# williamyang1991/VToonify

Measured on AMD Instinct MI355X. Metric: frames/sec at 1024x1024 VToonify-D inference, higher is better.
Workload: dtype bf16

## Files before the change

vtoonify_amd/csrc/style_ops.hip:

```cpp
#include "vt_common.hpp"

namespace {

__global__ void __launch_bounds__(256)
linear_kernel(float* __restrict__ y, int ld_y, const float* __restrict__ x, int ld_x,
              const float* __restrict__ W, const float* __restrict__ b, int rows, int in_dim,
              int out_dim, float w_scale, float b_scale, int act, float slope, float gain) {
    const int lane = threadIdx.x & 63;
    const int64_t wave = (int64_t)blockIdx.x * 4 + (threadIdx.x >> 6);
    const int64_t total = (int64_t)rows * out_dim;
    const int64_t wi = wave < total ? wave : total - 1;
    const int r = (int)(wi / out_dim), o = (int)(wi % out_dim);
    const float* xr = x + (int64_t)r * ld_x;
    const float* wr = W + (int64_t)o * in_dim;
    float acc = 0.0f;
    for (int i = lane; i < in_dim; i += 64) acc += xr[i] * wr[i];
    acc = wave_sum(acc);
    if (lane == 0 && wave < total) {
        float v = acc * w_scale;
        if (b) v += b[o] * b_scale;
        if (act == VT_ACT_LRELU) v = ((v > 0.0f) ? v : v * slope) * gain;
        else if (act == VT_ACT_SIGMOID) v = 1.0f / (1.0f + expf(-v));
        y[(int64_t)r * ld_y + o] = v;
    }
}

__global__ void __launch_bounds__(256)
pixel_norm_kernel(float* __restrict__ y, const float* __restrict__ x, int rows, int dim, const int* __restrict__ gate) {
    if (gate && gate[0] == 0) return;
    const int lane = threadIdx.x & 63;
    const int wave = blockIdx.x * 4 + (threadIdx.x >> 6);
    const int r = wave < rows ? wave : rows - 1;
    const float* xr = x + (int64_t)r * dim;
    float ss = 0.0f;
    for (int i = lane; i < dim; i += 64) ss += xr[i] * xr[i];
    ss = wave_sum(ss);
    const float inv = rsqrtf(ss / (float)dim + 1e-8f);
    if (wave < rows)
        for (int i = lane; i < dim; i += 64) y[(int64_t)r * dim + i] = xr[i] * inv;
}

template <typename T>
__global__ void __launch_bounds__(256)
modulate_weight_kernel(T* __restrict__ out, const float* __restrict__ w, const float* __restrict__ s,
                       int cout, int cin, int k, float scale, int demodulate,
                       const float* __restrict__ fir) {
    const int lane = threadIdx.x & 63;
    const int wave = blockIdx.x * 4 + (threadIdx.x >> 6);
    const int co = wave < cout ? wave : cout - 1;
    const bool live = wave < cout;
    const int taps = k * k;
    const int n = cin * taps;
    const float* wc = w + (int64_t)co * n;
    float demod = 1.0f;
    if (demodulate) {
        float ss = 0.0f;
        for (int i = lane; i < n; i += 64) {
            const float v = scale * wc[i] * s[i / taps];
            ss += v * v;
        }
        ss = wave_sum(ss);
        demod = rsqrtf(ss + 1e-8f);
    }
    if (!live) return;
    if (fir == nullptr) {
        T* oc = out + (int64_t)co * n;
        for (int i = lane; i < n; i += 64) {
            const int tap = i / cin, ci = i - tap * cin;
            const float v = scale * wc[ci * taps + tap] * s[ci] * demod;
            oc[i] = from_f32<T>(v);
        }
    } else {
        float K[16];
#pragma unroll
        for (int i = 0; i < 16; ++i) K[i] = fir[i];
        for (int ci = lane; ci < cin; ci += 64) {
            float wm[9];
#pragma unroll
            for (int t = 0; t < 9; ++t) wm[t] = scale * wc[ci * 9 + t] * s[ci] * demod;
#pragma unroll
            for (int p = 0; p < 4; ++p) {
                const int py = p >> 1, px = p & 1;
#pragma unroll
                for (int ky = 0; ky < 3; ++ky)
#pragma unroll
                    for (int kx = 0; kx < 3; ++kx) {
                        float acc = 0.0f;
#pragma unroll
                        for (int a = 0; a < 3; ++a) {
                            const int u = 4 - 2 * ky - a + py;
                            if (u < 0 || u > 3) continue;
#pragma unroll
                            for (int b = 0; b < 3; ++b) {
                                const int v = 4 - 2 * kx - b + px;
                                if (v < 0 || v > 3) continue;
                                acc += wm[a * 3 + b] * K[u * 4 + v];
                            }
                        }
                        out[((int64_t)(p * cout + co) * 9 + (ky * 3 + kx)) * cin + ci] = from_f32<T>(acc);
                    }
            }
        }
    }
}

constexpr int LIN_BATCH = 24, MOD_BATCH = 16;

struct LinearTable {
    vt_linear_item it[LIN_BATCH];
    const int* gate;
    int32_t first_wave[LIN_BATCH + 1];
    int32_t n;
};

__global__ void __launch_bounds__(256) linear_batch_kernel(const LinearTable t) {
    if (t.gate && t.gate[0] == 0) return;
    constexpr int RB = 6;
    const int lane = threadIdx.x & 63;
    const int wave = blockIdx.x * 4 + (threadIdx.x >> 6);
    __shared__ int pre[LIN_BATCH + 1];
    if (threadIdx.x <= (unsigned)t.n) pre[threadIdx.x] = t.first_wave[threadIdx.x];
    __syncthreads();
    const int total = pre[t.n];
    const int wv = wave < total ? wave : total - 1;
    int lo = 0, hi = t.n;
    while (hi - lo > 1) {
        const int mid = (lo + hi) >> 1;
        if (wv >= pre[mid]) lo = mid;
        else hi = mid;
    }
    const int k = lo;
    const vt_linear_item& L = t.it[k];
    const int o = wv - t.first_wave[k];
    const float* wr = L.W + (int64_t)o * L.in_dim;
    const bool quad = (L.in_dim % 4 == 0);
    const bool w16 = quad && ((uintptr_t)L.W % 16 == 0);
    const bool x16 = quad && (L.ld_x % 4 == 0) && ((uintptr_t)L.x % 16 == 0);
    for (int r0 = 0; r0 < L.rows; r0 += RB) {
        float acc[RB];
#pragma unroll
        for (int j = 0; j < RB; ++j) acc[j] = 0.0f;
        if (quad) {
            for (int i = lane * 4; i < L.in_dim; i += 256) {
                float w4[4];
                if (w16) {
                    unpack16<float>(ld128(wr + i), w4);
                } else {
                    w4[0] = wr[i]; w4[1] = wr[i + 1]; w4[2] = wr[i + 2]; w4[3] = wr[i + 3];
                }
#pragma unroll
                for (int j = 0; j < RB; ++j) {
                    const int r = (r0 + j < L.rows) ? r0 + j : L.rows - 1;
                    const float* xp = L.x + (int64_t)r * L.ld_x + i;
                    float x4[4];
                    if (x16) {
                        unpack16<float>(ld128(xp), x4);
                    } else {
                        x4[0] = xp[0]; x4[1] = xp[1]; x4[2] = xp[2]; x4[3] = xp[3];
                    }
                    acc[j] += (x4[0] * w4[0] + x4[1] * w4[1]) + (x4[2] * w4[2] + x4[3] * w4[3]);
                }
            }
        } else {
            for (int i = lane; i < L.in_dim; i += 64) {
                const float w = wr[i];
#pragma unroll
                for (int j = 0; j < RB; ++j) {
                    const int r = (r0 + j < L.rows) ? r0 + j : L.rows - 1;
                    acc[j] += L.x[(int64_t)r * L.ld_x + i] * w;
                }
            }
        }
#pragma unroll
        for (int j = 0; j < RB; ++j) acc[j] = wave_sum(acc[j]);
        if (lane == 0 && wave < total) {
#pragma unroll
            for (int j = 0; j < RB; ++j) {
                if (r0 + j >= L.rows) break;
                float v = acc[j] * L.w_scale;
                if (L.b) v += L.b[o] * L.b_scale;
                if (L.act == VT_ACT_LRELU) v = ((v > 0.0f) ? v : v * L.slope) * L.gain;
                else if (L.act == VT_ACT_SIGMOID) v = 1.0f / (1.0f + expf(-v));
                L.y[(int64_t)(r0 + j) * L.ld_y + o] = v;
            }
        }
    }
}

struct ModTable {
    vt_modulate_item it[MOD_BATCH];
    const int* gate;
    int32_t first_row[MOD_BATCH + 1];
    int32_t n;
};

template <typename T>
__global__ void __launch_bounds__(256) modulate_batch_kernel(const ModTable t) {
    if (t.gate && t.gate[0] == 0) return;
    __shared__ float red[4];
    const int tid = threadIdx.x, lane = tid & 63, wv = tid >> 6;
    int lo = 0, hi = t.n;
    while (hi - lo > 1) {
        const int mid = (lo + hi) >> 1;
        if ((int)blockIdx.x >= t.first_row[mid]) lo = mid;
        else hi = mid;
    }
    const int k = lo;
    const vt_modulate_item& M = t.it[k];
    const int co = blockIdx.x - t.first_row[k];
    const int cout = M.cout, cin = M.cin, taps = M.k * M.k;
    const int n = cin * taps;
    const float* w = (const float*)M.weight;
    const float* s = M.s;
    const float* wc = w + (int64_t)co * n;
    const float scale = M.scale;
    float demod = 1.0f;
    if (M.demodulate) {
        float ss = 0.0f;
        for (int i = tid; i < n; i += 256) {
            const float v = scale * wc[i] * s[i / taps];
            ss += v * v;
        }
        ss = wave_sum(ss);
        if (lane == 0) red[wv] = ss;
        __syncthreads();
        demod = rsqrtf(((red[0] + red[1]) + (red[2] + red[3])) + 1e-8f);
    }
    T* out = (T*)M.out;
    if (M.fir == nullptr) {
        T* oc = out + (int64_t)co * n;
        for (int i = tid; i < n; i += 256) {
            const int tap = i / cin, ci = i - tap * cin;
            oc[i] = from_f32<T>(scale * wc[ci * taps + tap] * s[ci] * demod);
        }
    } else {
        float K[16];
#pragma unroll
        for (int i = 0; i < 16; ++i) K[i] = M.fir[i];
        for (int ci = tid; ci < cin; ci += 256) {
            float wm[9];
#pragma unroll
            for (int q = 0; q < 9; ++q) wm[q] = scale * wc[ci * 9 + q] * s[ci] * demod;
#pragma unroll
            for (int p = 0; p < 4; ++p) {
                const int py = p >> 1, px = p & 1;
#pragma unroll
                for (int ky = 0; ky < 3; ++ky)
#pragma unroll
                    for (int kx = 0; kx < 3; ++kx) {
                        float acc = 0.0f;
#pragma unroll
                        for (int a = 0; a < 3; ++a) {
                            const int u = 4 - 2 * ky - a + py;
                            if (u < 0 || u > 3) continue;
#pragma unroll
                            for (int b = 0; b < 3; ++b) {
                                const int v = 4 - 2 * kx - b + px;
                                if (v < 0 || v > 3) continue;
                                acc += wm[a * 3 + b] * K[u * 4 + v];
                            }
                        }
                        out[((int64_t)(p * cout + co) * 9 + (ky * 3 + kx)) * cin + ci] = from_f32<T>(acc);
                    }
            }
        }
    }
}

template <typename T>
__global__ void __launch_bounds__(256)
pack_weight_kernel(T* __restrict__ out, const float* __restrict__ w, int cout, int cin_src, int kh,
                   int kw, int cin_dst, const int32_t* __restrict__ chan_map, float scale,
                   int src_transposed) {
    const int taps = kh * kw;
    const int64_t total = (int64_t)cout * taps * cin_dst;
    const int64_t stride = (int64_t)gridDim.x * 256;
    for (int64_t i = (int64_t)blockIdx.x * 256 + threadIdx.x; i < total; i += stride) {
        const int cd = (int)(i % cin_dst);
        const int64_t t = i / cin_dst;
        const int tap = (int)(t % taps);
        const int co = (int)(t / taps);
        const int cs = chan_map ? chan_map[cd] : (cd < cin_src ? cd : -1);
        float v = 0.0f;
        if (cs >= 0) {
            if (!src_transposed) {
                v = w[((int64_t)co * cin_src + cs) * taps + tap];
            } else {
                v = w[((int64_t)cs * cout + co) * taps + tap];
            }
        }
        out[i] = from_f32<T>(v * scale);
    }
}

}

extern "C" int vt_linear(float* y, int ld_y, const float* x, int ld_x, const float* W,
                         const float* b, int rows, int in_dim, int out_dim, float w_scale,
                         float b_scale, int act, float slope, float gain, vt_stream stream) {
    VT_REQUIRE(y && x && W, "vt_linear: null tensor");
    VT_REQUIRE(rows >= 0 && in_dim > 0 && out_dim > 0, "vt_linear: bad sizes");
    VT_REQUIRE(act == VT_ACT_NONE || act == VT_ACT_LRELU || act == VT_ACT_SIGMOID, "vt_linear: unsupported act %d", act);
    if (rows == 0) return VT_OK;
    const int64_t waves = (int64_t)rows * out_dim;
    VT_LAUNCH(linear_kernel, dim3((unsigned)((waves + 3) / 4)), dim3(256), stream, y, ld_y, x, ld_x,
              W, b, rows, in_dim, out_dim, w_scale, b_scale, act, slope, gain);
    return vt_check_launch("vt_linear");
}

extern "C" int vt_pixel_norm(float* y, const float* x, int rows, int dim, vt_stream stream) {
    VT_REQUIRE(y && x && rows >= 0 && dim > 0, "vt_pixel_norm: bad arguments");
    if (rows == 0) return VT_OK;
    VT_LAUNCH(pixel_norm_kernel, dim3((unsigned)((rows + 3) / 4)), dim3(256), stream, y, x, rows, dim, (const int*)nullptr);
    return vt_check_launch("vt_pixel_norm");
}

extern "C" int vt_modulate_weight(void* out, const float* weight, const float* s, int cout, int cin,
                                  int k, float scale, int demodulate, const float* fir,
                                  int out_dtype, vt_stream stream) {
    VT_REQUIRE(out && weight && s, "vt_modulate_weight: null tensor");
    VT_REQUIRE(cout > 0 && cin > 0 && (k == 1 || k == 3), "vt_modulate_weight: bad shape");
    VT_REQUIRE(!fir || k == 3, "vt_modulate_weight: polyphase fold needs a 3x3 kernel");
    dim3 grid((unsigned)((cout + 3) / 4)), block(256);
    if (out_dtype == VT_F32) {
        auto kf = modulate_weight_kernel<float>;
        VT_LAUNCH(kf, grid, block, stream, (float*)out, weight, s, cout, cin, k, scale, demodulate, fir);
    } else if (out_dtype == VT_BF16) {
        auto kf = modulate_weight_kernel<bf16_t>;
        VT_LAUNCH(kf, grid, block, stream, (bf16_t*)out, weight, s, cout, cin, k, scale, demodulate, fir);
    } else if (out_dtype == VT_F16) {
        auto kf = modulate_weight_kernel<f16_t>;
        VT_LAUNCH(kf, grid, block, stream, (f16_t*)out, weight, s, cout, cin, k, scale, demodulate, fir);
    } else {
        vt_set_error("vt_modulate_weight: unsupported dtype %d", out_dtype);
        return VT_ERR_UNSUPPORTED;
    }
    return vt_check_launch("vt_modulate_weight");
}

extern "C" int vt_pack_conv_weight(void* out, const float* w, int cout, int cin_src, int kh, int kw,
                                   int cin_dst, const int32_t* chan_map, float scale,
                                   int src_transposed, int out_dtype, vt_stream stream) {
    VT_REQUIRE(out && w, "vt_pack_conv_weight: null tensor");
    VT_REQUIRE(cout > 0 && cin_src > 0 && cin_dst > 0 && kh > 0 && kw > 0, "vt_pack_conv_weight: bad shape");
    const int64_t total = (int64_t)cout * kh * kw * cin_dst;
    int64_t blocks = (total + 255) / 256;
    if (blocks > 8192) blocks = 8192;
    dim3 grid((unsigned)blocks), block(256);
    if (out_dtype == VT_F32) {
        auto kf = pack_weight_kernel<float>;
        VT_LAUNCH(kf, grid, block, stream, (float*)out, w, cout, cin_src, kh, kw, cin_dst, chan_map, scale, src_transposed);
    } else if (out_dtype == VT_BF16) {
        auto kf = pack_weight_kernel<bf16_t>;
        VT_LAUNCH(kf, grid, block, stream, (bf16_t*)out, w, cout, cin_src, kh, kw, cin_dst, chan_map, scale, src_transposed);
    } else if (out_dtype == VT_F16) {
        auto kf = pack_weight_kernel<f16_t>;
        VT_LAUNCH(kf, grid, block, stream, (f16_t*)out, w, cout, cin_src, kh, kw, cin_dst, chan_map, scale, src_transposed);
    } else {
        vt_set_error("vt_pack_conv_weight: unsupported dtype %d", out_dtype);
        return VT_ERR_UNSUPPORTED;
    }
    return vt_check_launch("vt_pack_conv_weight");
}

static int linear_batch_impl(const vt_linear_item* items, int n_items, const int* gate, vt_stream stream);
extern "C" int vt_linear_batch(const vt_linear_item* items, int n_items, vt_stream stream) {
    return linear_batch_impl(items, n_items, nullptr, stream);
}
// ... 110 lines not shown
```

vtoonify_amd/engine.py:

```python
from __future__ import annotations

import ctypes as C
import math
import os
from typing import Dict, List, Optional, Tuple

import torch

from . import _lib
from . import kernels as K
from ._lib import ACT_LRELU, ACT_NONE, ACT_RELU_TANH, OUT_NCHW, OUT_NHWC

SQRT2 = math.sqrt(2.0)
N_LATENT = 18
_DIL = {1: 4, 2: 4, 3: 2, 4: 2, 5: 1, 6: 1}
SKIP_HDR = 64


def _pad8(c: int) -> int:
    return (c + 7) // 8 * 8


class _Plan:
    def __init__(self):
        self.bufs: Dict[str, torch.Tensor] = {}
        self.style_ops: List[Tuple] = []
        self.enc_ops: List[Tuple] = []
        self.gen_ops: List[Tuple] = []
        self.keep: list = []
        self.masks: List[torch.Tensor] = []
        self.graphs: dict = {}
        self.convs: list = []


class VToonifyEngine:
    supports_borrow = True

    def __init__(self, state_dict: Dict[str, torch.Tensor], backbone: str = "dualstylegan",
                 in_size: int = 256, dtype: torch.dtype = torch.bfloat16,
                 device: Optional[torch.device] = None, cache_styles: bool = False,
                 tile_hints: Optional[Dict[str, int]] = None, style_gate: bool = False, x3: bool = False,
                 fuse_rgb128: bool = True, fused_gate=True, fold_rgb_up: bool = True):
        assert backbone in ("dualstylegan", "toonify")
        assert dtype in (torch.bfloat16, torch.float16, torch.float32)
        self.backbone = backbone
        self.dual = backbone == "dualstylegan"
        self.in_size = in_size
        self.dtype = dtype
        self.dt = K.dt_code(dtype)
        self.x3 = bool(x3) and dtype == torch.float32
        self.dt_conv = K.VT_F32X3 if self.x3 else self.dt
        self.h16 = dtype in (torch.bfloat16, torch.float16)
        self.precision = ({torch.bfloat16: "bf16", torch.float16: "fp16"}[dtype] if self.h16 else
                          ("fp32x3" if self.x3 else "fp32_exact"))
        self.esz = 2 if self.h16 else 4
        any_t = next(iter(state_dict.values()))
        self.device = torch.device(device) if device is not None else any_t.device
        if self.device.type == "cuda" and self.device.index is None:
            self.device = torch.device("cuda", torch.cuda.current_device())
        self.lib = _lib.lib()
        if self.device.type != "cuda" and not _lib.is_emulation():
            raise _lib.VtError("VToonifyEngine needs a GPU device (no CPU path)")
        self.cache_styles = cache_styles
        self.fuse_rgb128 = bool(fuse_rgb128)
        self.fused_gate = fused_gate if fused_gate == "all" else bool(fused_gate)
        self.fold_rgb_up = bool(fold_rgb_up)
        self.style_gate = bool(style_gate)
        self.graph_first = os.environ.get("VT_GRAPH_FIRST", "1") != "0"
        self.use_upblur = True
        self.tile_hints: Dict[str, int] = dict(tile_hints or {})
        if not self.tile_hints and os.environ.get("VT_TILE_HINTS"):
            import json
            with open(os.environ["VT_TILE_HINTS"]) as f:
                self.tile_hints = {k: int(v) for k, v in json.load(f).items()}
        self.sd = {k: v.detach().to(self.device, torch.float32).contiguous() for k, v in state_dict.items()}
        self.g = "generator.generator." if self.dual else "generator."
        self.n_down = 0
        while f"encoder.{self.n_down}.0.weight" in self.sd:
            self.n_down += 1
        self.n_fuse = sum(1 for lvl in range(5) if 2 ** (5 + lvl) <= in_size)
        import collections
        self._plans: "collections.OrderedDict[tuple, _Plan]" = collections.OrderedDict()
        self.max_plans = max(1, int(os.environ.get("VT_MAX_PLANS", "12")))
        self._shape_seen: Dict[tuple, int] = {}
        self._pack_static()

    def _pack_static(self):
        sd, T = self.sd, self.dtype
        self.w: Dict[str, torch.Tensor] = {}
        for bi in range(self.n_down):
            for j in (0, 2):
                wsrc = sd[f"encoder.{bi}.{j}.weight"]
                cin_dst = self._kpad(wsrc.shape[1]) if j == 2 else None
                if self._stem32(bi):
                    cin_dst = 32
                self.w[f"encoder.{bi}.{j}"] = K.pack_conv_weight(wsrc, cin_dst=cin_dst, out_dtype=T)
        for ii in range(6):
            for nm in ("conv", "conv2"):
                key = f"encoder.{self.n_down}.{ii}.{nm}"
                self.w[key] = K.pack_conv_weight(sd[key + ".weight"], out_dtype=T)
        self.w["enc_rgb"] = K.pack_conv_weight(sd[f"encoder.{self.n_down + 1}.weight"], out_dtype=T)
        if self.dual:
            for ii in range(1, 7):
                for nm in ("conv", "conv2"):
                    w = sd[f"res.{ii}.{nm}.0.weight"]
                    scale = 1.0 / math.sqrt(w.shape[1] * w.shape[2] * w.shape[3])
                    self.w[f"res.{ii}.{nm}"] = K.pack_conv_weight(w, scale=scale, out_dtype=T)
        for fi in range(self.n_fuse):
            if self.dual:
                self.w[f"fusion_out.{fi}.conv"] = K.pack_conv_weight(sd[f"fusion_out.{fi}.conv.weight"], out_dtype=T)
                self.w[f"fusion_out.{fi}.conv2"] = K.pack_conv_weight(sd[f"fusion_out.{fi}.conv2.weight"], out_dtype=T)
            else:
                self.w[f"fusion_out.{fi}"] = K.pack_conv_weight(sd[f"fusion_out.{fi}.weight"], out_dtype=T)
            wsk = sd[f"fusion_skip.{fi}.weight"]
            c = wsk.shape[1] - 3
            cmap = torch.tensor([0, 1, 2] + [-1] * (SKIP_HDR - 3) + list(range(3, c + 3)), dtype=torch.int32,
                                device=self.device)
            self.w[f"fusion_skip.{fi}"] = K.pack_conv_weight(wsk, cin_dst=c + SKIP_HDR, chan_map=cmap, out_dtype=T)
        self.modw = {}
        for i in range(6, 16):
            self.modw[f"convs.{i}"] = sd[f"{self.g}convs.{i}.conv.weight"][0].contiguous()
        for i in range(3, 8):
            self.modw[f"to_rgbs.{i}"] = sd[f"{self.g}to_rgbs.{i}.conv.weight"][0].contiguous()
            self.w[f"to_rgbs.{i}.bias"] = sd[f"{self.g}to_rgbs.{i}.bias"].reshape(3).contiguous()
        self.fir_up = sd[f"{self.g}convs.6.conv.blur.kernel"].contiguous()
        self.fir_rgb = sd[f"{self.g}to_rgbs.3.upsample.kernel"].contiguous()
        if self.use_upblur:
            k = self.fir_up.detach().float().cpu()
            if not (k.shape == (4, 4) and float(k.sum()) != 0.0 and
                    torch.allclose(torch.outer(k.sum(1), k.sum(0)) / k.sum(), k, rtol=1e-5, atol=1e-7)):
                self.use_upblur = False
        self._wstream: Dict[int, torch.Tensor] = {}
        unit = 8 * (64 if self.h16 else 32)
        for key, wt in self.w.items():
            if wt.ndim == 3 and wt.shape[1] == 9 and wt.shape[2] % unit == 0 and wt.shape[0] % 8 == 0:
                st = K.conv_weight_stream(wt)
                if st is not None:
                    self._wstream[wt.data_ptr()] = st

    def _stem32(self, bi: int) -> bool:
        sd = self.sd
        w0, w2 = sd[f"encoder.{bi}.0.weight"], sd[f"encoder.{bi}.2.weight"]
        return (bi == 0 and self.h16 and w0.shape[1] <= 32 and w0.shape[0] == 32 and
                w2.shape[0] % 32 == 0 and w2.shape[0] <= 256)

    def _kpad(self, c: int) -> int:
        step = 64 if self.h16 else 32
        return (c + step - 1) // step * step

    def _buf(self, plan: _Plan, name: str, shape, dtype=None) -> torch.Tensor:
        t = torch.empty(shape, dtype=dtype or self.dtype, device=self.device)
        plan.bufs[name] = t
        return t

    @staticmethod
    def conv_signature(d) -> str:
        return (f"{d.h}x{d.w}:{d.c0 + d.c1}->{d.cout * d.phases}:k{d.kh}s{d.stride}d{d.dil}p{d.phases}"
                + (":nchw" if d.out_layout == OUT_NCHW else "") + (":up" if d.up_fir else ""))

    def _apply_hint(self, d):
        h = self.tile_hints.get(self.conv_signature(d))
        if h:
            d.tile_hint = int(h)
        return d

    def _op_conv(self, ops, plan, ref_macs=None, branch=0, join=False, entry=None, **kw):
        wt = kw.get("weight")
        if isinstance(wt, torch.Tensor) and wt.data_ptr() in self._wstream:
            kw["weight_stream"] = self._wstream[wt.data_ptr()]
        d = self._apply_hint(K.make_conv_desc(dtype=self.dt_conv, **kw))
        plan.keep.append(d)
        cin = d.c0 + d.c1
        m = d.n * d.out_h * d.out_w
        cout_t = d.cout * d.phases
        macs = m * cout_t * d.kh * d.kw * cin if ref_macs is None else ref_macs
        osz = 4 if d.out_dtype == K.VT_F32 else 2
        nbytes = (d.n * d.h * d.w * cin * self.esz + cout_t * d.kh * d.kw * cin * self.esz +
                  m * cout_t * osz * (2 if d.resid else 1))
        info = {"name": "conv", "kernel": "conv_igemm", "flops": 2 * macs, "bytes": nbytes, "cin": cin,
                "cout": cout_t, "m": m, "k": d.kh * d.kw * cin, "hw": (d.out_h, d.out_w),
                "sig": self.conv_signature(d)}
        if branch:
            info["branch"] = branch
        if join:
            info["join"] = True
        if entry is not None:
            info["form"] = entry[2]
            info["bytes"] += entry[3]
        plan.convs.append((d, info, ops, len(ops)))
        ops.append((self.lib.vt_conv2d, (C.byref(d),), info) if entry is None else (entry[0], (C.byref(d),) + tuple(entry[1]), info))

    def _conv_kind(self, **kw) -> int:
        wt = kw.get("weight")
        if isinstance(wt, torch.Tensor) and wt.data_ptr() in self._wstream:
            kw["weight_stream"] = self._wstream[wt.data_ptr()]
        d = self._apply_hint(K.make_conv_desc(dtype=self.dt_conv, **kw))
        d.splitk_ws, d.splitk_ws_bytes = 1 << 20, 1 << 40
        tile = self.lib.vt_conv2d_tile(C.byref(d))
        return tile // 100000000 if tile >= 0 else -1

    def _rgbup_resident(self, tile: int, n: int, ho: int, wo: int, cout: int) -> bool:
        if os.environ.get("VT_PATCH_PIPE", "")[:1] in ("0", "1") or os.environ.get("VT_BATCH_EXACT", "")[:1] == "1":
            return False
        kind, sk, bm, bn = tile // 100000000, (tile // 1000000) % 100, (tile // 1000) % 1000, tile % 1000
        return (kind == 1 and sk <= 1 and bm == 256 and bn == 64 and cout == 64 and
                n * ((ho + 15) // 16) * ((wo + 15) // 16) >= 2 * self._patchw_wgs())

    def _patchw_wgs(self) -> int:
        e = os.environ.get("VT_PATCHW_WGS", "")
        if e.isdigit() and int(e) > 0:
            return int(e)
        if self.device.type == "cuda":
            return torch.cuda.get_device_properties(self.device).multi_processor_count
        return 256

    def _op_linear(self, ops, y, ld_y, x, ld_x, W, b, rows, w_scale=1.0, b_scale=1.0, act=ACT_NONE,
                   slope=0.2, gain=1.0):
        out_dim, in_dim = W.shape
        ops.append((self.lib.vt_linear,
                    (C.c_void_p(K._ptr(y)), ld_y, C.c_void_p(K._ptr(x)), ld_x, C.c_void_p(W.data_ptr()),
                     C.c_void_p(b.data_ptr() if b is not None else 0), rows, in_dim, out_dim,
                     float(w_scale), float(b_scale), act, float(slope), float(gain)), "linear"))

    @staticmethod
    def _info(what):
        if isinstance(what, dict):
            return what
        return {"name": what, "kernel": what, "flops": 0, "bytes": 0}

    def _run(self, ops, stream, plan=None):
        for fn, args, what in ops:
            rc = fn(*args, stream)
            if rc != 0:
                raise _lib.VtError(f"{self._info(what)['name']} failed (code {rc}): "
                                   f"{self.lib.vt_last_error().decode()}")

    def _build_style_ops(self, plan: _Plan, ns: int, has_res: bool):
        sd, g, ops, lib = self.sd, self.g, plan.style_ops, self.lib
        f32 = torch.float32
        style_in = self._buf(plan, "style_in", (ns, N_LATENT, 512), f32)
        gate = None
        if self.style_gate:
            style_in.zero_()
            style_new = self._buf(plan, "style_new", (ns, N_LATENT, 512), f32)
            gflag = self._buf(plan, "style_gate", (2,), torch.int32)
            gflag[0], gflag[1] = 0, 1
            gate = C.c_void_p(gflag.data_ptr())
            ops.append((lib.vt_style_gate, (gate, C.c_void_p(style_in.data_ptr()), C.c_void_p(style_new.data_ptr()),
                                            ns * N_LATENT * 512), "style_gate"))
        ada = self._buf(plan, "adastyles", (ns, N_LATENT, 512), f32)
        ds = self._buf(plan, "d_s", (1,), f32)
        rows = ns * N_LATENT
        levels: List[list] = [[] for _ in range(5)]

        def lin(level, y, ld_y, x, ld_x, W, b, nrows, w_scale=1.0, b_scale=1.0, act=ACT_NONE, slope=0.2,
                gain=1.0):
            it = _lib.LinearItem()
            it.y, it.x, it.W = K._ptr(y), K._ptr(x), W.data_ptr()
            it.b = b.data_ptr() if b is not None else None
            it.ld_y, it.ld_x, it.rows = ld_y, ld_x, nrows
            it.out_dim, it.in_dim = W.shape
            it.act, it.w_scale, it.b_scale, it.slope, it.gain = act, w_scale, b_scale, slope, gain
            levels[level].append(it)

        if self.dual:
            pn = self._buf(plan, "pn", (rows, 512), f32)
            t1 = self._buf(plan, "tc1", (rows, 512), f32)
            res = self._buf(plan, "resstyles", (ns, N_LATENT, 512), f32)
            if gate is not None:
                ops.append((lib.vt_pixel_norm_gated, (C.c_void_p(pn.data_ptr()), C.c_void_p(style_in.data_ptr()), rows, 512,
                                                      gate), "pixel_norm"))
            else:
                ops.append((lib.vt_pixel_norm, (C.c_void_p(pn.data_ptr()), C.c_void_p(style_in.data_ptr()), rows, 512),
                            "pixel_norm"))
            sc = (1.0 / math.sqrt(512)) * 0.01
            lin(0, t1, 512, pn, 512, sd["generator.style.1.weight"], sd["generator.style.1.bias"],
                rows, sc, 0.01, ACT_LRELU, 0.2, SQRT2)
            lin(1, res, 512, t1, 512, sd["generator.style.2.weight"], sd["generator.style.2.bias"],
                rows, sc, 0.01, ACT_LRELU, 0.2, SQRT2)
            for i in range(7, N_LATENT):
                lin(0, ada.data_ptr() + i * 512 * 4, N_LATENT * 512, style_in.data_ptr() + i * 512 * 4,
                    N_LATENT * 512, sd[f"generator.res.{i}.weight"], sd[f"generator.res.{i}.bias"], ns,
                    1.0 / math.sqrt(512), 1.0)
        else:
            ops.append((self._copy_op, (ada, style_in), "copy"))

        plan.modw = {}
        mods = []
        for lvl in range(5):
            for name, lat, demod, up in ((f"convs.{6 + 2 * lvl}", 7 + 2 * lvl, True, True),
                                         (f"convs.{7 + 2 * lvl}", 8 + 2 * lvl, True, False),
                                         (f"to_rgbs.{3 + lvl}", 9 + 2 * lvl, False, False)):
                w = self.modw[name]
                cout, cin, k, _ = w.shape
                s = self._buf(plan, f"s.{name}", (ns, cin), f32)
                lin(1, s, cin, ada.data_ptr() + lat * 512 * 4, N_LATENT * 512,
                    sd[f"{g}{name}.conv.modulation.weight"], sd[f"{g}{name}.conv.modulation.bias"],
                    ns, 1.0 / math.sqrt(512), 1.0)
                phases = 4 if (up and not self.use_upblur) else 1
                taps = 9 if up else k * k
                wm = self._buf(plan, f"wm.{name}", (ns, phases * cout, taps, cin))
                plan.modw[name] = wm
                for b in range(ns):
                    it = _lib.ModulateItem()
                    it.out = wm.data_ptr() + b * phases * cout * taps * cin * self.esz
                    it.weight, it.s = w.data_ptr(), s.data_ptr() + b * cin * 4
                    it.fir = self.fir_up.data_ptr() if (up and not self.use_upblur) else None
                    it.cout, it.cin, it.k, it.demodulate = cout, cin, k, int(demod)
                    it.scale = 1.0 / math.sqrt(cin * k * k)
                    mods.append(it)
        if self.dual:
            if has_res:
                for ii in range(1, 7):
                    for nm in ("norm", "norm2"):
                        Wl = sd[f"res.{ii}.{nm}.style.weight"]
                        gb = self._buf(plan, f"gb.res.{ii}.{nm}", (ns, Wl.shape[0]), f32)
                        lin(2, gb, Wl.shape[0], plan.bufs["resstyles"].data_ptr() + ii * 512 * 4,
                            N_LATENT * 512, Wl, sd[f"res.{ii}.{nm}.style.bias"], ns)
            for fi in range(self.n_fuse):
                p = f"fusion_out.{fi}."
                l0 = self._buf(plan, f"lab0.{fi}", (ns, 64), f32)
                l1 = self._buf(plan, f"lab1.{fi}", (ns, 128), f32)
                lin(0, l0, 64, ds, 0, sd[p + "linear.0.weight"], sd[p + "linear.0.bias"], ns,
                    1.0, 1.0, ACT_LRELU, 0.2, 1.0)
                lin(1, l1, 128, l0, 64, sd[p + "linear.2.weight"], sd[p + "linear.2.bias"], ns,
                    1.0, 1.0, ACT_LRELU, 0.2, 1.0)
                Wl = sd[p + "norm.style.weight"]
                gb = self._buf(plan, f"gb.fus.{fi}", (ns, Wl.shape[0]), f32)
                lin(2, gb, Wl.shape[0], l1, 128, Wl, sd[p + "norm.style.bias"], ns)
        else:
            pass
        for lv in levels:
            if not lv:
                continue
            arr = (_lib.LinearItem * len(lv))(*lv)
            plan.keep.append(arr)
            linfo = {"name": "linear", "kernel": "linear_batch", "flops": 0, "bytes": 0}
            if gate is not None:
                ops.append((lib.vt_linear_batch_gated, (arr, len(lv), gate), linfo))
            else:
                ops.append((lib.vt_linear_batch, (arr, len(lv)), linfo))
        marr = (_lib.ModulateItem * len(mods))(*mods)
        plan.keep.append(marr)
        minfo = {"name": "modulate", "kernel": "modulate_batch", "flops": 0,
                 "bytes": sum(m.cout * m.cin * m.k * m.k * (4 + self.esz * (4 if m.fir else 1)) for m in mods)}
        if gate is not None:
            ops.append((lib.vt_modulate_weight_batch_gated, (marr, len(mods), self.dt, gate), minfo))
        else:
            ops.append((lib.vt_modulate_weight_batch, (marr, len(mods), self.dt), minfo))

    @staticmethod
    def _copy_op(dst, src, stream):
        dst.copy_(src)
        return 0

    @staticmethod
    def _fill_rows_op(dst, src, stream):
        dst.copy_(src.expand_as(dst))
        return 0

    def _build_plan(self, B: int, H: int, W: int, shared: bool, has_res: bool) -> _Plan:
        sd, g, lib, dt = self.sd, self.g, self.lib, self.dt
        plan = _Plan()
        ns = 1 if shared else B
        self._build_style_ops(plan, ns, has_res)
        f32 = torch.float32
        ops = plan.enc_ops
        ds = plan.bufs["d_s"]

        cin0 = sd["encoder.0.0.weight"].shape[1]
        cin_p = 32 if self._stem32(0) else _pad8(cin0)
        x_nhwc = self._buf(plan, "x_nhwc", (B, H, W, cin_p))
        if cin_p != _pad8(cin0):
            x_nhwc.zero_()
        plan.cin0 = cin0
        cur, cc, h, w = x_nhwc, cin_p, H, W
        feats = []
        for bi in range(self.n_down):
            stride = 1 if bi == 0 else 2
            for j in (0, 2):
                wt = sd[f"encoder.{bi}.{j}.weight"]
                co = wt.shape[0]
                st = stride if j == 0 else 1
                ho, wo = (h + 2 - 3) // st + 1, (w + 2 - 3) // st + 1
                cs = self._kpad(co) if (j == 0 and not self._stem32(bi)) else co
                out = self._buf(plan, f"enc{bi}.{j}", (B, ho, wo, cs))
                if cs != co:
                    out.zero_()
                self._op_conv(ops, plan, src0=cur, c0=cc, ld0=cc, n=B, h=h, w=w, out_h=ho, out_w=wo,
                              weight=self.w[f"encoder.{bi}.{j}"], cout=co, kh=3, kw=3, stride=st, pad=1,
                              bias=sd[f"encoder.{bi}.{j}.bias"], act=ACT_LRELU, slope=0.2, out=out, ld_out=cs)
                cur, cc, h, w = out, cs, ho, wo
            feats.append((cur, cc, h, w))
        feats = feats[::-1]
        cf = cc
        tmp = self._buf(plan, "res_tmp", (B, h, w, cf))
        ping = [self._buf(plan, "feat_a", (B, h, w, cf)), self._buf(plan, "feat_b", (B, h, w, cf))]
        hw = h * w
        if self.dual and has_res:
            sc1 = self._buf(plan, "in_scale", (B, cf), f32)
            sh1 = self._buf(plan, "in_shift", (B, cf), f32)
            ws = self._buf(plan, "in_ws", (max(K.instnorm_ws_bytes(B, hw, cf), 16),), torch.uint8)
            nrm_res = self._buf(plan, "nrm_res", (B, h, w, cf))
        feat = cur
        pp = 0
        rk = f"encoder.{self.n_down}"
        plane_adain = self.dual and has_res and hw <= 4096
        for ii in range(6):
            self._op_conv(ops, plan, src0=feat, c0=cf, ld0=cf, n=B, h=h, w=w, out_h=h, out_w=w,
                          weight=self.w[f"{rk}.{ii}.conv"], cout=cf, kh=3, kw=3, pad=1,
                          bias=sd[f"{rk}.{ii}.conv.bias"], act=ACT_LRELU, out=tmp, ld_out=cf)
            nxt = ping[pp]; pp ^= 1
            self._op_conv(ops, plan, src0=tmp, c0=cf, ld0=cf, n=B, h=h, w=w, out_h=h, out_w=w,
                          weight=self.w[f"{rk}.{ii}.conv2"], cout=cf, kh=3, kw=3, pad=1,
                          bias=sd[f"{rk}.{ii}.conv2.bias"], act=ACT_LRELU, alpha=1 / SQRT2, beta=1 / SQRT2,
                          resid=feat, ld_res=cf, out=nxt, ld_out=cf,
                          stats_part=ws if (self.dual and has_res and hw <= 16384 and not plane_adain) else None)
            feat = nxt
            if plane_adain:
                r = ii + 1
                dil = _DIL[r]
                gb1, gb2 = plan.bufs[f"gb.res.{r}.norm"], plan.bufs[f"gb.res.{r}.norm2"]
                ldg = 0 if ns == 1 else gb1.shape[1]

                def _plane(dst, src, gb):
                    ops.append((lib.vt_instnorm_plane,
                                (C.c_void_p(dst.data_ptr()), cf, C.c_void_p(src.data_ptr()), cf, C.c_void_p(0), 0, B, hw, cf,
                                 C.c_void_p(gb.data_ptr()), ldg, dt),
                                {"name": "adain", "kernel": "instnorm_plane", "flops": 0,
                                 "bytes": 2 * B * hw * cf * self.esz}))
                _plane(nrm_res, feat, gb1)
                self._op_conv(ops, plan, src0=nrm_res, c0=cf, ld0=cf, n=B, h=h, w=w, out_h=h, out_w=w,
                              weight=self.w[f"res.{r}.conv"], cout=cf, kh=3, kw=3, pad=dil, dil=dil,
                              bias=sd[f"res.{r}.conv.1.bias"], act=ACT_LRELU, gain=SQRT2, out=tmp, ld_out=cf)
                _plane(tmp, tmp, gb2)
                nxt = ping[pp]; pp ^= 1
                self._op_conv(ops, plan, src0=tmp, c0=cf, ld0=cf, n=B, h=h, w=w, out_h=h, out_w=w,
                              weight=self.w[f"res.{r}.conv2"], cout=cf, kh=3, kw=3, pad=dil, dil=dil,
                              bias=sd[f"res.{r}.conv2.1.bias"], act=ACT_LRELU, gain=SQRT2, alpha_dev=ds, beta=1.0,
                              resid=feat, ld_res=cf, out=nxt, ld_out=cf)
                feat = nxt
            elif self.dual and has_res:
                r = ii + 1
                dil = _DIL[r]
                for nm, src, dst in (("norm", feat, tmp), ("norm2", tmp, None)):
                    gb = plan.bufs[f"gb.res.{r}.{nm}"]
                    if hw <= 16384:
                        ops.append((lib.vt_instnorm_apply_stats,
                                    (C.c_void_p(nrm_res.data_ptr()), cf, C.c_void_p(src.data_ptr()), cf, B, hw, cf,
                                     C.c_void_p(gb.data_ptr()), 0 if ns == 1 else gb.shape[1],
                                     C.c_void_p(ws.data_ptr()), dt),
                                    {"name": "adain", "kernel": "instnorm_apply", "flops": 0,
                                     "bytes": 2 * B * hw * cf * self.esz}))
                    else:
                        ops.append((lib.vt_instnorm_stats,
                                    (C.c_void_p(sc1.data_ptr()), C.c_void_p(sh1.data_ptr()), C.c_void_p(src.data_ptr()),
                                     cf, C.c_void_p(0), 0, B, hw, cf, C.c_void_p(gb.data_ptr()),
                                     0 if ns == 1 else gb.shape[1], C.c_void_p(ws.data_ptr()), dt),
                                    {"name": "instnorm", "kernel": "instnorm_stats", "flops": 0,
                                     "bytes": B * hw * cf * self.esz}))
                        ops.append((lib.vt_affine_apply,
                                    (C.c_void_p(nrm_res.data_ptr()), cf, C.c_void_p(src.data_ptr()), cf,
                                     C.c_void_p(0), 0, C.c_void_p(sc1.data_ptr()), C.c_void_p(sh1.data_ptr()),
                                     B, hw, cf, dt),
                                    {"name": "affine", "kernel": "affine_apply", "flops": 0,
                                     "bytes": 2 * B * hw * cf * self.esz}))
                    cn = "conv" if nm == "norm" else "conv2"
                    if dst is not None:
                        self._op_conv(ops, plan, src0=nrm_res, c0=cf, ld0=cf, n=B, h=h, w=w, out_h=h, out_w=w,
                                      weight=self.w[f"res.{r}.{cn}"], cout=cf, kh=3, kw=3, pad=dil, dil=dil,
                                      bias=sd[f"res.{r}.{cn}.1.bias"],
                                      act=ACT_LRELU, gain=SQRT2, out=dst, ld_out=cf,
                                      stats_part=ws if hw <= 16384 else None)
                    else:
                        nxt = ping[pp]; pp ^= 1
                        self._op_conv(ops, plan, src0=nrm_res, c0=cf, ld0=cf, n=B, h=h, w=w, out_h=h, out_w=w,
                                      weight=self.w[f"res.{r}.{cn}"], cout=cf, kh=3, kw=3, pad=dil, dil=dil,
                                      bias=sd[f"res.{r}.{cn}.1.bias"],
                                      act=ACT_LRELU, gain=SQRT2, alpha_dev=ds, beta=1.0, resid=feat, ld_res=cf,
                                      out=nxt, ld_out=cf)
                        feat = nxt
        plan.feat = (feat, cf, h, w)
        skip = self._buf(plan, "skip_enc", (B, 3, h, w), f32)
        self._op_conv(ops, plan, src0=feat, c0=cf, ld0=cf, n=B, h=h, w=w, out_h=h, out_w=w,
# ... 370 lines not shown
```

Baseline: 1691.

## Trim style MLP to used rows and restructure linear/modulate style kernels

The style mapping MLP (pixel norm plus two linears) now runs only over the latent rows that the residual blocks read, instead of all 18 rows per sample. It is also skipped entirely when no residual path needs it. The batched linear kernel keeps small weight rows in registers, adds a single-row specialization, and spreads the final per-row writes across lanes. The modulate kernel stages the scaled weights in shared memory so that non-FIR rows are read once for both the demod sum and the output. The style stage is cheap relative to the generator, so the overall effect on frame rate is likely small.

```diff
diff --git a/vtoonify_amd/csrc/style_ops.hip b/vtoonify_amd/csrc/style_ops.hip
--- a/vtoonify_amd/csrc/style_ops.hip
+++ b/vtoonify_amd/csrc/style_ops.hip
@@ -113,6 +113,93 @@
     int32_t n;
 };
 
+__device__ __forceinline__ float fmul(float a, float b) {
+#ifdef VT_EMU
+    return a * b;
+#else
+    return __fmul_rn(a, b);
+#endif
+}
+__device__ __forceinline__ float fadd(float a, float b) {
+#ifdef VT_EMU
+    return a + b;
+#else
+    return __fadd_rn(a, b);
+#endif
+}
+__device__ __forceinline__ float dot4(const float (&x)[4], const float (&w)[4]) {
+    return fadd(fadd(fmul(x[0], w[0]), fmul(x[1], w[1])), fadd(fmul(x[2], w[2]), fmul(x[3], w[3])));
+}
+__device__ __forceinline__ void ld_quad(float (&v)[4], const float* p, bool vec) {
+    if (vec) {
+        unpack16<float>(ld128(p), v);
+    } else {
+        v[0] = p[0]; v[1] = p[1]; v[2] = p[2]; v[3] = p[3];
+    }
+}
+
+template <int NR>
+__device__ __forceinline__ void linear_rows(const vt_linear_item& L, const float* wr, const float (&wq)[2][4], bool wregs,
+                                            float bias, int o, int r0, int lane, bool live, bool quad, bool w16, bool x16) {
+    float acc[NR];
+    const float* xr[NR];
+#pragma unroll
+    for (int j = 0; j < NR; ++j) {
+        acc[j] = 0.0f;
+        const int r = (r0 + j < L.rows) ? r0 + j : L.rows - 1;
+        xr[j] = L.x + (int64_t)r * L.ld_x;
+    }
+    if (wregs) {
+        float xq[2][NR][4];
+#pragma unroll
+        for (int s = 0; s < 2; ++s) {
+            const int i = lane * 4 + 256 * s;
+            if (i < L.in_dim) {
+#pragma unroll
+                for (int j = 0; j < NR; ++j) ld_quad(xq[s][j], xr[j] + i, x16);
+            }
+        }
+#pragma unroll
+        for (int s = 0; s < 2; ++s) {
+            if (lane * 4 + 256 * s < L.in_dim) {
+#pragma unroll
+                for (int j = 0; j < NR; ++j) acc[j] = fadd(acc[j], dot4(xq[s][j], wq[s]));
+            }
+        }
+    } else if (quad) {
+        for (int i = lane * 4; i < L.in_dim; i += 256) {
+            float w4[4], x4[NR][4];
+            ld_quad(w4, wr + i, w16);
+#pragma unroll
+            for (int j = 0; j < NR; ++j) ld_quad(x4[j], xr[j] + i, x16);
+#pragma unroll
+            for (int j = 0; j < NR; ++j) acc[j] = fadd(acc[j], dot4(x4[j], w4));
+        }
+    } else {
+        for (int i = lane; i < L.in_dim; i += 64) {
+            const float w = wr[i];
+            float x1[NR];
+#pragma unroll
+            for (int j = 0; j < NR; ++j) x1[j] = xr[j][i];
+#pragma unroll
+            for (int j = 0; j < NR; ++j) acc[j] = fadd(acc[j], fmul(x1[j], w));
+        }
+    }
+#pragma unroll
+    for (int j = 0; j < NR; ++j) acc[j] = wave_sum(acc[j]);
+    float mine = acc[0];
+#pragma unroll
+    for (int j = 1; j < NR; ++j)
+        if (lane == j) mine = acc[j];
+    if (live && lane < NR && r0 + lane < L.rows) {
+        float v = fmul(mine, L.w_scale);
+        if (L.b) v = fadd(v, fmul(bias, L.b_scale));
+        if (L.act == VT_ACT_LRELU) v = fmul((v > 0.0f) ? v : fmul(v, L.slope), L.gain);
+        else if (L.act == VT_ACT_SIGMOID) v = 1.0f / (1.0f + expf(-v));
+        L.y[(int64_t)(r0 + lane) * L.ld_y + o] = v;
+    }
+}
+
 __global__ void __launch_bounds__(256) linear_batch_kernel(const LinearTable t) {
     if (t.gate && t.gate[0] == 0) return;
     constexpr int RB = 6;
@@ -122,68 +209,34 @@
     if (threadIdx.x <= (unsigned)t.n) pre[threadIdx.x] = t.first_wave[threadIdx.x];
     __syncthreads();
     const int total = pre[t.n];
-    const int wv = wave < total ? wave : total - 1;
+    const int wv = vt_uniform(wave < total ? wave : total - 1);
     int lo = 0, hi = t.n;
     while (hi - lo > 1) {
         const int mid = (lo + hi) >> 1;
         if (wv >= pre[mid]) lo = mid;
         else hi = mid;
     }
-    const int k = lo;
+    const int k = vt_uniform(lo);
     const vt_linear_item& L = t.it[k];
     const int o = wv - t.first_wave[k];
     const float* wr = L.W + (int64_t)o * L.in_dim;
     const bool quad = (L.in_dim % 4 == 0);
     const bool w16 = quad && ((uintptr_t)L.W % 16 == 0);
     const bool x16 = quad && (L.ld_x % 4 == 0) && ((uintptr_t)L.x % 16 == 0);
+    const bool live = wave < total;
+    const bool wregs = quad && L.in_dim <= 512;
+    float wq[2][4] = {};
+    if (wregs) {
+#pragma unroll
+        for (int s = 0; s < 2; ++s) {
+            const int i = lane * 4 + 256 * s;
+            if (i < L.in_dim) ld_quad(wq[s], wr + i, w16);
+        }
+    }
+    const float bias = L.b ? L.b[o] : 0.0f;
     for (int r0 = 0; r0 < L.rows; r0 += RB) {
-        float acc[RB];
-#pragma unroll
-        for (int j = 0; j < RB; ++j) acc[j] = 0.0f;
-        if (quad) {
-            for (int i = lane * 4; i < L.in_dim; i += 256) {
-                float w4[4];
-                if (w16) {
-                    unpack16<float>(ld128(wr + i), w4);
-                } else {
-                    w4[0] = wr[i]; w4[1] = wr[i + 1]; w4[2] = wr[i + 2]; w4[3] = wr[i + 3];
-                }
-#pragma unroll
-                for (int j = 0; j < RB; ++j) {
-                    const int r = (r0 + j < L.rows) ? r0 + j : L.rows - 1;
-                    const float* xp = L.x + (int64_t)r * L.ld_x + i;
-                    float x4[4];
-                    if (x16) {
-                        unpack16<float>(ld128(xp), x4);
-                    } else {
-                        x4[0] = xp[0]; x4[1] = xp[1]; x4[2] = xp[2]; x4[3] = xp[3];
-                    }
-                    acc[j] += (x4[0] * w4[0] + x4[1] * w4[1]) + (x4[2] * w4[2] + x4[3] * w4[3]);
-                }
-            }
-        } else {
-            for (int i = lane; i < L.in_dim; i += 64) {
-                const float w = wr[i];
-#pragma unroll
-                for (int j = 0; j < RB; ++j) {
-                    const int r = (r0 + j < L.rows) ? r0 + j : L.rows - 1;
-                    acc[j] += L.x[(int64_t)r * L.ld_x + i] * w;
-                }
-            }
-        }
-#pragma unroll
-        for (int j = 0; j < RB; ++j) acc[j] = wave_sum(acc[j]);
-        if (lane == 0 && wave < total) {
-#pragma unroll
-            for (int j = 0; j < RB; ++j) {
-                if (r0 + j >= L.rows) break;
-                float v = acc[j] * L.w_scale;
-                if (L.b) v += L.b[o] * L.b_scale;
-                if (L.act == VT_ACT_LRELU) v = ((v > 0.0f) ? v : v * L.slope) * L.gain;
-                else if (L.act == VT_ACT_SIGMOID) v = 1.0f / (1.0f + expf(-v));
-                L.y[(int64_t)(r0 + j) * L.ld_y + o] = v;
-            }
-        }
+        if (L.rows - r0 == 1) linear_rows<1>(L, wr, wq, wregs, bias, o, r0, lane, live, quad, w16, x16);
+        else linear_rows<RB>(L, wr, wq, wregs, bias, o, r0, lane, live, quad, w16, x16);
     }
 }
 
@@ -194,10 +247,61 @@
     int32_t n;
 };
 
+constexpr int MOD_STAGE = 4608;
+constexpr int MOD_PER_THREAD = MOD_STAGE / 256;
+
+template <typename T>
+__device__ __forceinline__ void modulate_row_staged(T* __restrict__ oc, const float* __restrict__ wc, const float* __restrict__ s,
+                                                    int cin, int taps, float scale, int demodulate, float* stage, float* red) {
+    const int tid = threadIdx.x, lane = tid & 63, wv = tid >> 6;
+    const int n = cin * taps;
+    const int dq = 256 / taps, dr = 256 - dq * taps;
+    float wreg[MOD_PER_THREAD], sreg[MOD_PER_THREAD];
+    {
+        int ci = tid / taps, tap = tid - ci * taps;
+#pragma unroll
+        for (int j = 0; j < MOD_PER_THREAD; ++j) {
+            const int i = tid + 256 * j;
+            if (256 * j >= n) break;
+            if (i < n) {
+                wreg[j] = wc[i];
+                sreg[j] = s[ci];
+            }
+            ci += dq, tap += dr;
+            if (tap >= taps) tap -= taps, ++ci;
+        }
+    }
+    float ss = 0.0f;
+#pragma unroll
+    for (int j = 0; j < MOD_PER_THREAD; ++j) {
+        const int i = tid + 256 * j;
+        if (256 * j >= n) break;
+        if (i < n) {
+            const float v = fmul(fmul(scale, wreg[j]), sreg[j]);
+            stage[i] = v;
+            ss = fadd(ss, fmul(v, v));
+        }
+    }
+    if (demodulate) {
+        ss = wave_sum(ss);
+        if (lane == 0) red[wv] = ss;
+    }
+    __syncthreads();
+    const float demod = demodulate ? rsqrtf(fadd(fadd(fadd(red[0], red[1]), fadd(red[2], red[3])), 1e-8f)) : 1.0f;
+    const int eq = 256 / cin, er = 256 - eq * cin;
+    int tap = tid / cin, ci = tid - tap * cin;
+    for (int i = tid; i < n; i += 256) {
+        oc[i] = from_f32<T>(fmul(stage[ci * taps + tap], demod));
+        tap += eq, ci += er;
+        if (ci >= cin) ci -= cin, ++tap;
+    }
+}
+
 template <typename T>
 __global__ void __launch_bounds__(256) modulate_batch_kernel(const ModTable t) {
     if (t.gate && t.gate[0] == 0) return;
     __shared__ float red[4];
+    __shared__ float stage[MOD_STAGE];
     const int tid = threadIdx.x, lane = tid & 63, wv = tid >> 6;
     int lo = 0, hi = t.n;
     while (hi - lo > 1) {
@@ -214,6 +318,10 @@
     const float* s = M.s;
     const float* wc = w + (int64_t)co * n;
     const float scale = M.scale;
+    if (M.fir == nullptr && n <= MOD_STAGE) {
+        modulate_row_staged<T>((T*)M.out + (int64_t)co * n, wc, s, cin, taps, scale, M.demodulate, stage, red);
+        return;
+    }
     float demod = 1.0f;
     if (M.demodulate) {
         float ss = 0.0f;
diff --git a/vtoonify_amd/engine.py b/vtoonify_amd/engine.py
--- a/vtoonify_amd/engine.py
+++ b/vtoonify_amd/engine.py
@@ -15,6 +15,7 @@
 N_LATENT = 18
 _DIL = {1: 4, 2: 4, 3: 2, 4: 2, 5: 1, 6: 1}
 SKIP_HDR = 64
+LIN_BATCH = 24
 
 
 def _pad8(c: int) -> int:
@@ -40,7 +41,8 @@
                  in_size: int = 256, dtype: torch.dtype = torch.bfloat16,
                  device: Optional[torch.device] = None, cache_styles: bool = False,
                  tile_hints: Optional[Dict[str, int]] = None, style_gate: bool = False, x3: bool = False,
-                 fuse_rgb128: bool = True, fused_gate=True, fold_rgb_up: bool = True):
+                 fuse_rgb128: bool = True, fused_gate=True, fold_rgb_up: bool = True,
+                 trim_style_rows: bool = True):
         assert backbone in ("dualstylegan", "toonify")
         assert dtype in (torch.bfloat16, torch.float16, torch.float32)
         self.backbone = backbone
@@ -65,6 +67,7 @@
         self.fuse_rgb128 = bool(fuse_rgb128)
         self.fused_gate = fused_gate if fused_gate == "all" else bool(fused_gate)
         self.fold_rgb_up = bool(fold_rgb_up)
+        self.trim_style_rows = bool(trim_style_rows)
         self.style_gate = bool(style_gate)
         self.graph_first = os.environ.get("VT_GRAPH_FIRST", "1") != "0"
         self.use_upblur = True
@@ -253,31 +256,26 @@
         rows = ns * N_LATENT
         levels: List[list] = [[] for _ in range(5)]
 
-        def lin(level, y, ld_y, x, ld_x, W, b, nrows, w_scale=1.0, b_scale=1.0, act=ACT_NONE, slope=0.2,
-                gain=1.0):
+        def item(y, ld_y, x, ld_x, W, b, nrows, w_scale=1.0, b_scale=1.0, act=ACT_NONE, slope=0.2, gain=1.0):
             it = _lib.LinearItem()
             it.y, it.x, it.W = K._ptr(y), K._ptr(x), W.data_ptr()
             it.b = b.data_ptr() if b is not None else None
             it.ld_y, it.ld_x, it.rows = ld_y, ld_x, nrows
             it.out_dim, it.in_dim = W.shape
             it.act, it.w_scale, it.b_scale, it.slope, it.gain = act, w_scale, b_scale, slope, gain
-            levels[level].append(it)
-
-        if self.dual:
+            return it
+
+        def lin(level, *a, **kw):
+            levels[level].append(item(*a, **kw))
+
+        res_rows: List[int] = []
+        mlp_at = len(ops)
+        want_mlp = self.dual and (has_res or not self.trim_style_rows)
+        if want_mlp:
             pn = self._buf(plan, "pn", (rows, 512), f32)
             t1 = self._buf(plan, "tc1", (rows, 512), f32)
             res = self._buf(plan, "resstyles", (ns, N_LATENT, 512), f32)
-            if gate is not None:
-                ops.append((lib.vt_pixel_norm_gated, (C.c_void_p(pn.data_ptr()), C.c_void_p(style_in.data_ptr()), rows, 512,
-                                                      gate), "pixel_norm"))
-            else:
-                ops.append((lib.vt_pixel_norm, (C.c_void_p(pn.data_ptr()), C.c_void_p(style_in.data_ptr()), rows, 512),
-                            "pixel_norm"))
-            sc = (1.0 / math.sqrt(512)) * 0.01
-            lin(0, t1, 512, pn, 512, sd["generator.style.1.weight"], sd["generator.style.1.bias"],
-                rows, sc, 0.01, ACT_LRELU, 0.2, SQRT2)
-            lin(1, res, 512, t1, 512, sd["generator.style.2.weight"], sd["generator.style.2.bias"],
-                rows, sc, 0.01, ACT_LRELU, 0.2, SQRT2)
+        if self.dual:
             for i in range(7, N_LATENT):
                 lin(0, ada.data_ptr() + i * 512 * 4, N_LATENT * 512, style_in.data_ptr() + i * 512 * 4,
                     N_LATENT * 512, sd[f"generator.res.{i}.weight"], sd[f"generator.res.{i}.bias"], ns,
@@ -312,10 +310,11 @@
         if self.dual:
             if has_res:
                 for ii in range(1, 7):
+                    res_rows.append(ii)
                     for nm in ("norm", "norm2"):
                         Wl = sd[f"res.{ii}.{nm}.style.weight"]
                         gb = self._buf(plan, f"gb.res.{ii}.{nm}", (ns, Wl.shape[0]), f32)
-                        lin(2, gb, Wl.shape[0], plan.bufs["resstyles"].data_ptr() + ii * 512 * 4,
+                        lin(2, gb, Wl.shape[0], res.data_ptr() + ii * 512 * 4,
                             N_LATENT * 512, Wl, sd[f"res.{ii}.{nm}.style.bias"], ns)
             for fi in range(self.n_fuse):
                 p = f"fusion_out.{fi}."
@@ -330,6 +329,20 @@
                 lin(2, gb, Wl.shape[0], l1, 128, Wl, sd[p + "norm.style.bias"], ns)
         else:
             pass
+        if want_mlp:
+            lo, n_span = (min(res_rows), max(res_rows) - min(res_rows) + 1) if res_rows else (0, 0)
+            trim = self.trim_style_rows and (ns == 1 or all(len(levels[lv]) + ns <= LIN_BATCH for lv in (0, 1)))
+            spans = [(b * N_LATENT + lo, n_span) for b in range(ns)] if trim else [(0, rows)]
+            p0, p1 = spans[0][0], spans[-1][0] + spans[-1][1]
+            pn_args = (C.c_void_p(pn.data_ptr() + p0 * 512 * 4), C.c_void_p(style_in.data_ptr() + p0 * 512 * 4), p1 - p0, 512)
+            if gate is not None:
+                ops.insert(mlp_at, (lib.vt_pixel_norm_gated, pn_args + (gate,), "pixel_norm"))
+            else:
+                ops.insert(mlp_at, (lib.vt_pixel_norm, pn_args, "pixel_norm"))
+            sc = (1.0 / math.sqrt(512)) * 0.01
+            for lv, y, x, nm in ((0, t1, pn, "generator.style.1"), (1, res, t1, "generator.style.2")):
+                levels[lv][0:0] = [item(y.data_ptr() + r0 * 512 * 4, 512, x.data_ptr() + r0 * 512 * 4, 512, sd[nm + ".weight"],
+                                        sd[nm + ".bias"], nr, sc, 0.01, ACT_LRELU, 0.2, SQRT2) for r0, nr in spans]
         for lv in levels:
             if not lv:
                 continue
```

New measurement: 1703 (median of 6 runs). Within noise of the previous version (+0.7%).
